# MoZhou1995/DeepPDE_ActorCritic

Hardware: AMD Instinct MI355X
Metric: SDE trajectory-steps/sec (batch×horizon) at d=20; value-fn rel-L2 vs analytic (higher is better)
Workload: dtype f32

## Files before the change

### deeppde_actorcritic_amd/csrc/dpac_device.h

```cpp
#pragma once

#include <hip/hip_runtime.h>
#include <rocrand/rocrand_kernel.h>
#include <stdint.h>

#include <type_traits>

#include "dpac.h"
#include "dpac_mfma.h"

namespace dpac {

__host__ __device__ constexpr int pow2_at_least(int v) {
  int p = 1;
  while (p < v) p *= 2;
  return p;
}
#ifndef DPAC_LANE_CAP
#define DPAC_LANE_CAP 16
#endif
#ifndef DPAC_LANE_COMPS
#define DPAC_LANE_COMPS 2
#endif
__host__ __device__ constexpr int lanes_for_dim(int D) {
// ... 216 lines not shown
  return __builtin_bit_cast(float, (unsigned)sw[0]) + __builtin_bit_cast(float, (unsigned)sw[1]);
}
__device__ __forceinline__ double row_pair_sum(double v) {
  const unsigned long long u = __builtin_bit_cast(unsigned long long, v);
  const unsigned lo = (unsigned)u, hi = (unsigned)(u >> 32);
  const auto sl = __builtin_amdgcn_permlane16_swap(lo, lo, false, false);
  const auto sh = __builtin_amdgcn_permlane16_swap(hi, hi, false, false);
  const double a = __builtin_bit_cast(double, ((unsigned long long)(unsigned)sh[0] << 32) | (unsigned)sl[0]);
  const double b = __builtin_bit_cast(double, ((unsigned long long)(unsigned)sh[1] << 32) | (unsigned)sl[1]);
  return a + b;
}

template <int P, typename T>
__device__ __forceinline__ T group_shift_in(T keep, T v, bool group_start) {
  if constexpr (P == 1) {
    return v;
  } else {
    constexpr int kRowShr1 = 0x111;
    T sh;
    if constexpr (sizeof(T) == 4) {
      sh = __builtin_bit_cast(T, __builtin_amdgcn_update_dpp(__builtin_bit_cast(int, v),
                                                            __builtin_bit_cast(int, keep),
                                                            kRowShr1, 0xF, 0xF, false));
    } else {
      const long long vb = __builtin_bit_cast(long long, v), kb = __builtin_bit_cast(long long, keep);
      const int lo = __builtin_amdgcn_update_dpp((int)vb, (int)kb, kRowShr1, 0xF, 0xF, false);
      const int hi = __builtin_amdgcn_update_dpp((int)(vb >> 32), (int)(kb >> 32), kRowShr1, 0xF, 0xF,
                                                 false);
      sh = __builtin_bit_cast(T, ((long long)hi << 32) | (unsigned int)lo);
    }
    if constexpr (P < 16) sh = group_start ? v : sh;
    return sh;
  }
}

template <typename T>
__device__ __forceinline__ void pin(T& v) {
  asm volatile("" : "+v"(v));
}
template <typename T, typename... Ts>
__device__ __forceinline__ void pin(T& v, Ts&... more) {
  pin(v);
  pin(more...);
}

template <int P>
struct Lanes {
  static_assert(P == 1 || P == 2 || P == 4 || P == 8 || P == 16 || P == 32, "bad group size");
  template <typename T>
  __device__ __forceinline__ static T sum(T v) {
    if constexpr (P >= 2) v = v + dpp<kDppXor1>(v);
    if constexpr (P >= 4) v = v + dpp<kDppXor2>(v);
    if constexpr (P >= 8) v = v + dpp<kDppHalfMirror>(v);
    if constexpr (P >= 16) v = v + dpp<kDppMirror>(v);
    if constexpr (P >= 32) v = row_pair_sum(v);
    return v;
  }
};

enum : uint64_t { kTagDw = 0, kTagDir = 1, kTagRadius = 2, kTagBdry = 3 };

__device__ __forceinline__ uint4 philox_block(uint64_t seed, uint64_t subseq, uint64_t block) {
  rocrand_state_philox4x32_10 st;
  rocrand_init(seed, subseq, block * 4ull, &st);
  return rocrand4(&st);
}

__device__ __forceinline__ void box_muller_hw(unsigned int x, unsigned int y, float& a, float& b) {
  const float u = ROCRAND_2POW32_INV + (x * ROCRAND_2POW32_INV);
  const float v = ROCRAND_2POW32_INV_2PI + (y * ROCRAND_2POW32_INV_2PI);
  const float s = __builtin_amdgcn_sqrtf(-2.0f * __logf(u));
  float sn, cs;
  __sincosf(v, &sn, &cs);
  a = sn * s;
  b = cs * s;
}
// ... 385 lines not shown
  __device__ __forceinline__ void drift_vjp(const T (&x)[M], const T (&u)[MC], T r, const T (&a)[M],
                            T (&gx)[M], T (&gu)[MC]) const {
#pragma unroll
    for (int i = 0; i < C; ++i) {
      const T x1 = x[i], x2 = x[C + i], a1 = a[i], a2v = a[C + i];
      gx[i] += a2v * (-2 * x1 * x2 - 1);
      gx[C + i] += a1 + a2v * (1 - x1 * x1);
      gu[i] += a2v;
    }
  }
  __device__ __forceinline__ void sigma_vjp(const T (&x)[M], const T (&u)[MC], const T (&a)[M], T (&gx)[M],
                            T (&gu)[MC]) const {}
  __device__ __forceinline__ void w_vjp(const T (&x)[M], const T (&u)[MC], T gw, T (&gx)[M], T (&gu)[MC]) const {
    T dv1[C], dv2[C], g[C], Ldv2[C], Lg[C];
    Lop(x, dv1);
    Lop(x + C, dv2);
#pragma unroll
    for (int i = 0; i < C; ++i) g[i] = (1 - x[i] * x[i]) * x[C + i] - x[i];
    Lop(dv2, Ldv2);
    Lop(g, Lg);
#pragma unroll
    for (int i = 0; i < C; ++i) {
      const T x1 = x[i], x2 = x[C + i];
      const T s1 = x[nxt(i)] + x[prv(i)], s2 = x[C + nxt(i)] + x[C + prv(i)];
      const T d1 = geps * s1 + 2 * x1 * x2 * dv2[i] + two_ga * x1;
      const T d2 = geps * s2 + Ldv2[i] * inv2q - dv1[i] - (1 - x1 * x1) * dv2[i] - Lg[i] + two_ga * x2;
      gx[i] += gw * d1;
      gx[C + i] += gw * d2;
      gu[i] += gw * (two_q * u[i]);
    }
  }
};

template <class E>
struct ConstSigma : std::false_type {};
template <typename T, int D, int P>
struct ConstSigma<EqLQR<T, D, P>> : std::true_type {};
template <typename T, int D, int P>
struct ConstSigma<EqEKN<T, D, P>> : std::true_type {};

}
```

### deeppde_actorcritic_amd/csrc/dpac_kernels.h

```cpp
#pragma once

#include <cmath>
#include <limits>
#include <type_traits>
#include <utility>

#include "dpac_device.h"

namespace dpac {

enum Op : int {
  OP_ROLLOUT = 0,
  OP_FLAG_INIT,
  OP_STEP_FWD,
  OP_STEP_BWD,
  OP_TD_FWD,
  OP_TD_BWD,
  OP_EVAL,
  OP_ROLLOUT_NN,
  OP_ROLLOUT_NN_BWD,
};

inline int nn_mask_tile_bytes(int n_hidden) { return 13 * 64 * n_hidden; }

struct OpArgs {
  int op;
  dpac_eqn_params eq;
  int scheme, dtype, td_type, cost_order, sample_type, what;
  int64_t B, traj_offset;
  int N;
  double T;
  uint64_t seed;
  const void *x0, *dw, *x, *u, *dt_in, *coef_in, *G, *disc_in, *y_in;
  const int32_t* flag_in;
  const void *g_x_out, *g_disc_out, *g_y_out;
  void *x_out, *dt, *coef, *u_out, *y, *disc, *disc_out, *y_out;
  int32_t* flag_out;
  void *g_x, *g_u, *g_disc, *g_G, *out;
  dpac_mlp mlp;
  void *save_z, *save_disc;
// ... 330 lines not shown
    if constexpr (WANT_U) su.store(rs_u, u, (uint32_t)t * slab_u);
    if constexpr (DPAC_ABLATE != 3) {
      constexpr int PH = decltype(phase)::value;
      keep = group_shift_in<P>(keep, tr.coef ? tr.dt : -tr.dt, lc.p == 0);
      if constexpr (PH >= 0) {
        if constexpr (PH % F == F - 1) flush(t, F);
      } else if ((t & (F - 1)) == F - 1) {
        flush(t, F);
      }
    }
  };
  pipelined<KB, DwFrame<T, M>>(0, a.N, load, body);
  if constexpr (DPAC_ABLATE != 3 && DPAC_ABLATE != 1 && DPAC_ABLATE != 5) {
    const int rem = a.N & (F - 1);
    if (rem) flush(a.N - 1, rem);
  }
  if constexpr (COST) {
    if (lc.live && lc.p == 0) {
      a.y[lc.b] = y;
      a.disc[lc.b] = disc;
    }
  }
}

#ifndef DPAC_ST_CHUNKS
#define DPAC_ST_CHUNKS 4
#endif
#ifndef DPAC_ST_TIGHT
#define DPAC_ST_TIGHT 0
#endif
#ifndef DPAC_ST_TIGHT_CHUNKS
#define DPAC_ST_TIGHT_CHUNKS 3
#endif
#ifndef DPAC_ST_PD
#define DPAC_ST_PD 1
#endif
constexpr int kStCW = 4;
constexpr int kStCH = 16;
constexpr int kStPD = DPAC_ST_PD;
#ifndef DPAC_ST_STEP
#define DPAC_ST_STEP 1
#endif
constexpr bool kOwnStep = DPAC_ST_STEP != 0;
static_assert(kStPD >= 1 && kStPD <= kStCH, "prefetch distance within a chunk");
template <typename T, int D, int P>
struct StagedPlan {
  static constexpr int TPW = kStCW * (64 / P);
  static constexpr int SLOT = TPW * D * (int)sizeof(T);
  static constexpr int PIECES = (SLOT + 1023) / 1024;
  static constexpr int kLdsCap = 128 * 1024;
  static constexpr int SLOT_1K = (SLOT + 16 + 1023) / 1024 * 1024;
  static constexpr int SLOT_16 = (SLOT + 16 + 15) / 16 * 16;
  static constexpr bool kWide = !DPAC_ST_TIGHT && DPAC_ST_CHUNKS * kStCH * SLOT_1K <= kLdsCap;
  static constexpr int CHUNKS = kWide ? DPAC_ST_CHUNKS : DPAC_ST_TIGHT_CHUNKS;
  static constexpr int SLOT_LDS = kWide ? SLOT_1K : SLOT_16;
  static constexpr int PADOFF = SLOT_LDS - 16;
  static constexpr int RS = CHUNKS * kStCH;
  static_assert(P < 4 || (SLOT % 16 == 0 && (PIECES - 1) * 1024 + 16 <= SLOT), "DMA pieces stay inside the slot");
  static constexpr bool kOk = P >= 4 && RS * SLOT_LDS <= kLdsCap && kStCH * PIECES <= 62;
};

template <class Fn, int... S>
__device__ __forceinline__ void unroll_phases(Fn& fn, std::integer_sequence<int, S...>) {
  (fn(Phase<S>{}), ...);
}

__device__ __forceinline__ int lds_load_relaxed(const int* p) {
  return __hip_atomic_load(p, __ATOMIC_RELAXED, __HIP_MEMORY_SCOPE_WORKGROUP);
}
__device__ __forceinline__ void lds_store_relaxed(int* p, int v) {
  __hip_atomic_store(p, v, __ATOMIC_RELAXED, __HIP_MEMORY_SCOPE_WORKGROUP);
}

template <int GEN>
constexpr int st_waves() { return kStCW + (GEN > 0 ? GEN : 1); }
#ifndef DPAC_ST_GEN
#define DPAC_ST_GEN 12
#endif
constexpr int kStGen = DPAC_ST_GEN;

#ifndef DPAC_ST_TRACE
#define DPAC_ST_TRACE 0
#endif
#if DPAC_ST_TRACE
constexpr int kStTraceRow = 128, kStTraceWaves = 16, kStTraceChunks = 32;
static __device__ uint32_t g_st_trace[2 * kStTraceWaves * kStTraceRow];
__device__ __forceinline__ uint32_t st_clock() {
  unsigned long long t;
  __builtin_amdgcn_sched_barrier(0);
  asm volatile("s_memtime %0\n\ts_waitcnt lgkmcnt(0)" : "=s"(t)::"memory");
  __builtin_amdgcn_sched_barrier(0);
  return (uint32_t)t;
}
__device__ __forceinline__ uint32_t st_realtime() {
  unsigned long long t;
  __builtin_amdgcn_sched_barrier(0);
  asm volatile("s_memrealtime %0\n\ts_waitcnt lgkmcnt(0)" : "=s"(t)::"memory");
  __builtin_amdgcn_sched_barrier(0);
  return (uint32_t)t;
}
#define ST_PUT(pt, v)                \
  do {                               \
    const uint32_t st_v_ = (v);      \
    if (st_on) st_row[(pt)] = st_v_; \
  } while (0)
#define ST_MARK(pt) ST_PUT(pt, st_clock())
#define ST_CHUNK(base, c0) ((base) + ((c0) / kStCH < kStTraceChunks ? (c0) / kStCH : kStTraceChunks - 1))
#else
#define ST_PUT(pt, v) \
  do {                \
  } while (0)
#define ST_MARK(pt) \
  do {              \
  } while (0)
#endif

template <typename T, class E, int D, int SCHEME, int OUT, int KB, int GEN = 0>
__global__ __launch_bounds__(64 * st_waves<GEN>()) void k_rollout_staged(const E eq, const DevConsts<T> c,
                                                                          const RolloutArgs<T> a) {
  constexpr int P = E::kP, M = E::M, MC = E::MC;
  using PL = StagedPlan<T, D, P>;
  constexpr int TPW = PL::TPW, RS = PL::RS, PIECES = PL::PIECES, SLOT_LDS = PL::SLOT_LDS;
  constexpr bool COST = (OUT & kOutCost) != 0, WANT_U = (OUT & kOutU) != 0;
  constexpr int F = P < kStCH ? P : kStCH;
  constexpr int NREADY = GEN > 0 ? GEN : 1;
  static_assert(kStCH % F == 0 && (F & (F - 1)) == 0, "flush phase fixed per unrolled body");
  static_assert(GEN == 0 || (2 * M <= 4 && kStCH % 2 == 0), "generators draw the paired layout");
  using TR = Transition<T, E, SCHEME>;
  __shared__ __attribute__((aligned(16))) unsigned char s_ring[RS * SLOT_LDS];
  __shared__ int s_ready[NREADY], s_done[kStCW];
  const int wave = __builtin_amdgcn_readfirstlane((int)threadIdx.x / 64), lane = (int)threadIdx.x % 64;
  const int64_t row0 = xcd_block(blockIdx.x, gridDim.x) * TPW;
  const int N = a.N;
#if DPAC_ST_TRACE
  const bool st_on = lane == 0 && wave < kStTraceWaves && (blockIdx.x == 0 || blockIdx.x == gridDim.x - 1);
  uint32_t* const st_row = g_st_trace + ((blockIdx.x == 0 ? 0 : kStTraceWaves) + (wave < kStTraceWaves ? wave : 0)) * kStTraceRow;
  ST_MARK(0);
  ST_PUT(5, st_realtime());
#endif
  if (threadIdx.x == 0) {
#pragma unroll
    for (int w = 0; w < NREADY; ++w) s_ready[w] = 0;
#pragma unroll
    for (int w = 0; w < kStCW; ++w) s_done[w] = 0;
  }
  if (threadIdx.x < RS * 4)
    reinterpret_cast<uint32_t*>(s_ring + (threadIdx.x / 4) * SLOT_LDS + PL::PADOFF)[threadIdx.x % 4] = 0u;
  __syncthreads();
  ST_MARK(1);

  if constexpr (GEN > 0) {
    if (wave >= kStCW) {
      const int g = wave - kStCW;
      const int64_t rows_live = (a.B - row0) < TPW ? (a.B - row0) : TPW;
      constexpr int PLS = (D + M - 1) / M;
      constexpr int NBLK = (kStCH / 2) * TPW * PLS;
      constexpr int PASSES = (NBLK + 64 * GEN - 1) / (64 * GEN);
      constexpr int SLOT_T = SLOT_LDS / (int)sizeof(T);
      T* const ringw = reinterpret_cast<T*>(s_ring);
      for (int c0 = 0; c0 < N; c0 += kStCH) {
        const int need = c0 + kStCH - RS;
        if (need > 0) {
          for (;;) {
            int mn = lds_load_relaxed(&s_done[0]);
#pragma unroll
            for (int w = 1; w < kStCW; ++w) mn = min(mn, lds_load_relaxed(&s_done[w]));
            if (mn >= need) break;
            __builtin_amdgcn_s_sleep(2);
          }
        }
        asm volatile("" ::: "memory");
#pragma unroll 1
        for (int k = 0; k < PASSES; ++k) {
          const int e = (k * GEN + g) * 64 + lane;
          const int u = e / (TPW * PLS), rem = e - u * (TPW * PLS);
          const int i = rem / PLS, p = rem - i * PLS;
          const int t0 = c0 + 2 * u;
          if (e < NBLK && t0 < N && i < rows_live) {
            T v[4];
            dw_block_values<T>(a.seed, (uint64_t)(a.traj_offset + row0 + i), (uint64_t)(t0 >> 1) * P + p,
                               a.sample_type, v);
            T* d0 = ringw + (t0 % RS) * SLOT_T + i * D + p * M;
            T* d1 = ringw + ((t0 + 1) % RS) * SLOT_T + i * D + p * M;
#pragma unroll
            for (int m = 0; m < M; ++m) {
              if (p * M + m < D) {
                d0[m] = v[m];
                if (t0 + 1 < N) d1[m] = v[M + m];
              }
            }
          }
        }
        asm volatile("s_waitcnt lgkmcnt(0)" ::: "memory");
        if (lane == 0) lds_store_relaxed(&s_ready[g], c0 + kStCH < N ? c0 + kStCH : N);
      }
      return;
    }
  } else if (wave == kStCW) {
    const int64_t rows_live = (a.B - row0) < TPW ? (a.B - row0) : TPW;
    const uint32_t bytes = (uint32_t)(rows_live * D * (int64_t)sizeof(T));
    const uint32_t lds0 = (uint32_t)(uintptr_t)(__attribute__((address_space(3))) unsigned char*)s_ring;
    const char* base = (const char*)(a.dw + row0 * D);
    const int64_t step_bytes = a.B * D * (int64_t)sizeof(T);
    for (int c0 = 0; c0 < N; c0 += kStCH) {
      const int need = c0 + kStCH - RS;
      if (need > 0) {
        for (;;) {
          int mn = lds_load_relaxed(&s_done[0]);
#pragma unroll
          for (int w = 1; w < kStCW; ++w) mn = min(mn, lds_load_relaxed(&s_done[w]));
          if (mn >= need) break;
          __builtin_amdgcn_s_sleep(2);
        }
      }
      asm volatile("" ::: "memory");
#if DPAC_ST_TRACE
      ST_MARK(ST_CHUNK(16, c0));
#endif
#pragma unroll
      for (int s = 0; s < kStCH; ++s) {
        const int t = c0 + s < N ? c0 + s : N - 1;
        const char* src = base + t * step_bytes;
        const uint32_t slot = lds0 + (uint32_t)((t % RS) * SLOT_LDS);
#pragma unroll
        for (int k = 0; k < PIECES; ++k) {
          const uint32_t off = (uint32_t)((k * 64 + lane) * 16);
          const char* gp = src + (off < bytes ? off : 0u);
          const uint32_t m0 = __builtin_amdgcn_readfirstlane(slot + (uint32_t)(k * 1024));
          if (off < bytes || lane == 0) {
            int keep;
            asm volatile("s_mov_b32 %0, m0\n\ts_mov_b32 m0, %2\n\ts_nop 0\n\tglobal_load_lds_dwordx4 %1, off\n\ts_mov_b32 m0, %0"
                         : "=&s"(keep) : "v"(gp), "s"(m0) : "memory");
          }
        }
      }
#if DPAC_ST_TRACE
      ST_MARK(ST_CHUNK(48, c0));
#endif
      if (c0 > 0) {
        asm volatile("s_waitcnt vmcnt(%0)" ::"n"(kStCH * PIECES) : "memory");
        if (lane == 0) lds_store_relaxed(&s_ready[0], c0);
#if DPAC_ST_TRACE
        ST_MARK(ST_CHUNK(80, c0));
#endif
      }
    }
    asm volatile("s_waitcnt vmcnt(0)" ::: "memory");
    if (lane == 0) lds_store_relaxed(&s_ready[0], N);
    ST_MARK(4);
    ST_PUT(6, st_realtime());
    return;
  }

  const LaneCoord<P> lc(a.B, lane, row0 + wave * (64 / P));
  const int gl = wave * (64 / P) + lane / P;
  const Own<D, P> own(lc.p);
  const Own<E::CDIM, P> ownu(lc.p);
  const BufSlab<T, D, P> sx(own, lc.b, lc.live);
  const BufSlab<T, E::CDIM, P> su(ownu, lc.b, lc.live);
  const uint32_t slab = (uint32_t)(a.B * D * sizeof(T));
  const uint32_t slab_u = (uint32_t)(a.B * E::CDIM * sizeof(T));
  const uint32_t row_bytes = (uint32_t)(N * sizeof(T));
  const __amdgpu_buffer_rsrc_t rs_x = make_rsrc(a.x, slab * (uint32_t)(N + 1));
  const __amdgpu_buffer_rsrc_t rs_u = make_rsrc(a.u, WANT_U ? slab_u * (uint32_t)N : 0u);
  const __amdgpu_buffer_rsrc_t rs_dt = make_rsrc(a.dt, (uint32_t)a.B * row_bytes);
  const __amdgpu_buffer_rsrc_t rs_cf = make_rsrc(a.coef, (uint32_t)a.B * row_bytes);
  const T* ring = reinterpret_cast<const T*>(s_ring);
  const int lds_e = gl * D + lc.p * M;
  constexpr bool kVecRead = Own<D, P>::kFull && (M * sizeof(T) == 8 || M * sizeof(T) == 16);
  const uint32_t lane_off = own.active() ? (uint32_t)(lds_e * (int)sizeof(T)) : (uint32_t)PL::PADOFF;
  T keep = 0;
  auto flush = [&](int t_last, int count) {
    const uint32_t off = (lc.live && lc.p < count)
                             ? (uint32_t)((lc.b * N + t_last - lc.p) * (int64_t)sizeof(T)) : kOOB;
    buf_store_scalar<T>(rs_dt, off, fabs(keep));
    buf_store_scalar<T>(rs_cf, off, keep > T(0) ? T(1) : T(0));
  };
  T x[M];
  sx.load(make_rsrc(a.x0, slab), x);
  sx.store(rs_x, x);
  T r = TR::kRadius ? dsqrt(Lanes<P>::sum(sumsq(x))) : T(0);
  Flags fl = SCHEME == DPAC_SCHEME_ADAPTIVE ? region(r, c) : Flags{true, false};
  T disc = 1, y = 0;
  T xc[M], rc = r;
#pragma unroll
  for (int m = 0; m < M; ++m) xc[m] = x[m];
  T Ra = fl.alive ? c.R : -std::numeric_limits<T>::infinity();
  bool alive = fl.alive;
  const T sq0 = SCHEME == DPAC_SCHEME_ADAPTIVE ? dsqrt(c.dt0) : c.sqrt_dt0;
  T dt = c.dt0, sq = sq0;
  if constexpr (kOwnStep && SCHEME == DPAC_SCHEME_ADAPTIVE) {
    dt = adaptive_dt_raw(fl.layer, r, c);
    dt = fl.layer ? fmax(dt, c.dt_min) : dt;
    sq = dsqrt(dt);
  }
  ST_MARK(2);
  auto read_dw_at = [&](int t, uint32_t slot_bytes, T (&dwv)[M]) {
    if constexpr (kVecRead) {
      typedef T vec __attribute__((ext_vector_type(M)));
      const vec v = *reinterpret_cast<const vec*>(s_ring + slot_bytes + lane_off);
#pragma unroll
      for (int m = 0; m < M; ++m) dwv[m] = v[m];
    } else {
      const T* slot = ring + (t % RS) * (SLOT_LDS / (int)sizeof(T)) + lds_e;
#pragma unroll
      for (int m = 0; m < M; ++m) dwv[m] = own.valid(m) ? slot[m] : T(0);
    }
  };
  auto read_dw = [&](int t, T (&dwv)[M]) { read_dw_at(t, (uint32_t)((t % RS) * SLOT_LDS), dwv); };
  auto body = [&](int t, const T (&dwv)[M], auto phase) {
    T u[MC];
    eq.u_true(x, r, u);
// ... 45 lines not shown
    } else {
      if constexpr (E::kNeedsNorm) rt = dsqrt(St);
      coef = alive && !(St - c.R2 >= T(0));
      alive = coef;
    }
    if constexpr (COST) {
      const T cf = coef ? T(1) : T(0);
      const T w = eq.w_finish(Lanes<P>::sum(eq.w_part(x, u)));
      y += cost_increment(a.cost_order, w, cf, dt, disc);
      disc = disc * disc_factor(dt, cf, c);
    }
    const T kv = coef ? dt : -dt;
#pragma unroll
    for (int m = 0; m < M; ++m) {
      x[m] = coef ? xt[m] : x[m];
      xc[m] = xt[m];
    }
    if constexpr (E::kNeedsNorm) {
      r = coef ? rt : r;
      rc = rt;
    }
    dt = dtn;
    sq = sqn;
    sx.template store<DPAC_ROLLOUT_X_AUX>(rs_x, x, (uint32_t)(t + 1) * slab);
    if constexpr (WANT_U) su.store(rs_u, u, (uint32_t)t * slab_u);
    constexpr int PH = decltype(phase)::value;
    keep = group_shift_in<P>(keep, kv, lc.p == 0);
    if constexpr (PH >= 0) {
      if constexpr (PH % F == F - 1) flush(t, F);
    } else if ((t & (F - 1)) == F - 1) {
      flush(t, F);
    }
  };
  for (int c0 = 0; c0 < N; c0 += kStCH) {
    const int want = c0 + kStCH < N ? c0 + kStCH : N;
#if DPAC_ST_TRACE
    const uint32_t st_poll0 = st_clock();
#endif
    for (;;) {
      int mn = lds_load_relaxed(&s_ready[0]);
#pragma unroll
      for (int w = 1; w < NREADY; ++w) mn = min(mn, lds_load_relaxed(&s_ready[w]));
      if (mn >= want) break;
      __builtin_amdgcn_s_sleep(1);
    }
    asm volatile("" ::: "memory");
#if DPAC_ST_TRACE
    {
      const uint32_t st_now = st_clock();
      ST_PUT(ST_CHUNK(16, c0), st_now);
      ST_PUT(ST_CHUNK(80, c0), st_now - st_poll0);
      if (c0 == 0) ST_PUT(3, st_now);
    }
#endif
    if (c0 + kStCH <= N) {
      const uint32_t cb = (uint32_t)__builtin_amdgcn_readfirstlane((c0 % RS) * SLOT_LDS);
      constexpr int PD = kStPD;
      T nxt[PD][M];
#pragma unroll
      for (int q = 0; q < PD; ++q) read_dw_at(c0 + q, cb + (uint32_t)(q * SLOT_LDS), nxt[q]);
      auto one = [&](auto sidx) {
        constexpr int S = decltype(sidx)::value;
        T cur[M];
#pragma unroll
        for (int m = 0; m < M; ++m) cur[m] = nxt[S % PD][m];
        if constexpr (S + PD < kStCH) read_dw_at(c0 + S + PD, cb + (uint32_t)((S + PD) * SLOT_LDS), nxt[S % PD]);
        if constexpr (PD > 1) __builtin_amdgcn_sched_barrier(0);
        if constexpr (kOwnStep)
          step(c0 + S, cur, Phase<S>{});
        else
          body(c0 + S, cur, Phase<S>{});
      };
      unroll_phases(one, std::make_integer_sequence<int, kStCH>{});
    } else {
      for (int t = c0; t < N; ++t) {
        T cur[M];
        read_dw(t, cur);
        if constexpr (kOwnStep)
          step(t, cur, Phase<-1>{});
        else
          body(t, cur, Phase<-1>{});
      }
    }
    asm volatile("s_waitcnt lgkmcnt(0)" ::: "memory");
    if (lane == 0) lds_store_relaxed(&s_done[wave], want);
#if DPAC_ST_TRACE
    ST_MARK(ST_CHUNK(48, c0));
#endif
  }
  const int rem = N & (F - 1);
  if (rem) flush(N - 1, rem);
#if DPAC_ST_TRACE
  ST_MARK(4);
  asm volatile("s_waitcnt vmcnt(0)" ::: "memory");
  ST_MARK(7);
  ST_PUT(6, st_realtime());
#endif
  if constexpr (COST) {
    if (lc.live && lc.p == 0) {
      a.y[lc.b] = y;
      a.disc[lc.b] = disc;
    }
  }
}

template <typename T, class E, int D, int SCHEME>
__global__ __launch_bounds__(64) void k_flag_init(const E eq, const DevConsts<T> c, int64_t B,
                                                   const T* x0, int32_t* flag) {
  constexpr int P = E::kP, M = E::M;
  const LaneCoord<P> lc(B, threadIdx.x, xcd_block(blockIdx.x, gridDim.x) * (64 / P));
  const Own<D, P> own(lc.p);
  T xv[M];
  own.load_masked(x0 + lc.b * D, xv);
  const T r = dsqrt(Lanes<P>::sum(sumsq(xv)));
  if (lc.p == 0) flag[lc.b] = SCHEME == DPAC_SCHEME_ADAPTIVE ? region(r, c).encode() : 1;
}

template <typename T>
struct StepArgs {
  int64_t B;
  int cost_order;
// ... 725 lines not shown
```

Measured before the change: 27.50 billion.

## Restructure staged rollout loader and consumer into grouped DMA issue with seamless chunk handoff

The loader wave now issues dw DMA in sub-groups of four steps using precomputed voffsets and a fast full-tile path that skips per-lane bounds checks and m0 save/restore. It also publishes readiness at finer granularity during the first chunks. The compute waves replace the per-chunk blocking poll with a seam loop that prefetches the next step's dw across chunk boundaries and polls readiness early. The aim is to shorten pipeline startup and hide chunk-boundary stalls, at the cost of more complex synchronisation and a requirement of at least three ring chunks. Some unused helpers are also removed.

Result: no change. 27.49 billion (-0.0%).

```diff
diff --git a/deeppde_actorcritic_amd/csrc/dpac_device.h b/deeppde_actorcritic_amd/csrc/dpac_device.h
--- a/deeppde_actorcritic_amd/csrc/dpac_device.h
+++ b/deeppde_actorcritic_amd/csrc/dpac_device.h
@@ -272,16 +272,6 @@
     if constexpr (P < 16) sh = group_start ? v : sh;
     return sh;
   }
-}
-
-template <typename T>
-__device__ __forceinline__ void pin(T& v) {
-  asm volatile("" : "+v"(v));
-}
-template <typename T, typename... Ts>
-__device__ __forceinline__ void pin(T& v, Ts&... more) {
-  pin(v);
-  pin(more...);
 }
 
 template <int P>
@@ -733,11 +723,4 @@
   }
 };
 
-template <class E>
-struct ConstSigma : std::false_type {};
-template <typename T, int D, int P>
-struct ConstSigma<EqLQR<T, D, P>> : std::true_type {};
-template <typename T, int D, int P>
-struct ConstSigma<EqEKN<T, D, P>> : std::true_type {};
-
-}
+}
diff --git a/deeppde_actorcritic_amd/csrc/dpac_kernels.h b/deeppde_actorcritic_amd/csrc/dpac_kernels.h
--- a/deeppde_actorcritic_amd/csrc/dpac_kernels.h
+++ b/deeppde_actorcritic_amd/csrc/dpac_kernels.h
@@ -6,6 +6,7 @@
 #include <utility>
 
 #include "dpac_device.h"
+#include "dpac_staged_sched.h"
 
 namespace dpac {
 
@@ -413,6 +414,18 @@
 #endif
 constexpr bool kOwnStep = DPAC_ST_STEP != 0;
 static_assert(kStPD >= 1 && kStPD <= kStCH, "prefetch distance within a chunk");
+#ifndef DPAC_ST_ISSUE
+#define DPAC_ST_ISSUE 1
+#endif
+#ifndef DPAC_ST_SUB
+#define DPAC_ST_SUB 1
+#endif
+#ifndef DPAC_ST_SEAM
+#define DPAC_ST_SEAM 1
+#endif
+constexpr bool kStIssue = DPAC_ST_ISSUE != 0, kStSub = DPAC_ST_SUB != 0, kStSeam = DPAC_ST_SEAM != 0;
+static_assert(stsched::kCH == kStCH, "the schedule header's chunk is the kernel's");
+static_assert(!kStSeam || kStPD == 1, "the seam loop carries one step of dw across the boundary");
 template <typename T, int D, int P>
 struct StagedPlan {
   static constexpr int TPW = kStCW * (64 / P);
@@ -448,6 +461,7 @@
 #define DPAC_ST_GEN 12
 #endif
 constexpr int kStGen = DPAC_ST_GEN;
+static_assert(64 * st_waves<kStGen>() <= 1024, "the Philox variant's workgroup (compute waves + generators) fits a 1024-thread block");
 
 #ifndef DPAC_ST_TRACE
 #define DPAC_ST_TRACE 0
@@ -496,6 +510,7 @@
   constexpr int NREADY = GEN > 0 ? GEN : 1;
   static_assert(kStCH % F == 0 && (F & (F - 1)) == 0, "flush phase fixed per unrolled body");
   static_assert(GEN == 0 || (2 * M <= 4 && kStCH % 2 == 0), "generators draw the paired layout");
+  static_assert(!kStSeam || stsched::ring_ok(PL::CHUNKS), "a wave waits for chunk c + 1 before it marks chunk c done");
   using TR = Transition<T, E, SCHEME>;
   __shared__ __attribute__((aligned(16))) unsigned char s_ring[RS * SLOT_LDS];
   __shared__ int s_ready[NREADY], s_done[kStCW];
@@ -567,54 +582,103 @@
       return;
     }
   } else if (wave == kStCW) {
+    using SC = stsched::Loader<PIECES, kStSub>;
+    constexpr int SUB = stsched::kSub, GROUPS = stsched::kGroups;
     const int64_t rows_live = (a.B - row0) < TPW ? (a.B - row0) : TPW;
     const uint32_t bytes = (uint32_t)(rows_live * D * (int64_t)sizeof(T));
     const uint32_t lds0 = (uint32_t)(uintptr_t)(__attribute__((address_space(3))) unsigned char*)s_ring;
-    const char* base = (const char*)(a.dw + row0 * D);
+    const char* const base = (const char*)(a.dw + row0 * D);
     const int64_t step_bytes = a.B * D * (int64_t)sizeof(T);
-    for (int c0 = 0; c0 < N; c0 += kStCH) {
-      const int need = c0 + kStCH - RS;
-      if (need > 0) {
-        for (;;) {
-          int mn = lds_load_relaxed(&s_done[0]);
-#pragma unroll
-          for (int w = 1; w < kStCW; ++w) mn = min(mn, lds_load_relaxed(&s_done[w]));
-          if (mn >= need) break;
-          __builtin_amdgcn_s_sleep(2);
-        }
-      }
-      asm volatile("" ::: "memory");
-#if DPAC_ST_TRACE
-      ST_MARK(ST_CHUNK(16, c0));
-#endif
-#pragma unroll
-      for (int s = 0; s < kStCH; ++s) {
-        const int t = c0 + s < N ? c0 + s : N - 1;
-        const char* src = base + t * step_bytes;
-        const uint32_t slot = lds0 + (uint32_t)((t % RS) * SLOT_LDS);
-#pragma unroll
-        for (int k = 0; k < PIECES; ++k) {
-          const uint32_t off = (uint32_t)((k * 64 + lane) * 16);
-          const char* gp = src + (off < bytes ? off : 0u);
-          const uint32_t m0 = __builtin_amdgcn_readfirstlane(slot + (uint32_t)(k * 1024));
-          if (off < bytes || lane == 0) {
-            int keep;
-            asm volatile("s_mov_b32 %0, m0\n\ts_mov_b32 m0, %2\n\ts_nop 0\n\tglobal_load_lds_dwordx4 %1, off\n\ts_mov_b32 m0, %0"
-                         : "=&s"(keep) : "v"(gp), "s"(m0) : "memory");
+    auto dma_fast = [](const char* src, uint32_t voff, uint32_t m0) {
+      asm volatile("s_mov_b32 m0, %2\n\ts_nop 0\n\tglobal_load_lds_dwordx4 %0, %1" ::"v"(voff), "s"(src), "s"(m0) : "memory");
+    };
+    auto dma_any = [&](const char* src, int k, uint32_t m0) {
+      const uint32_t off = (uint32_t)((k * 64 + lane) * 16);
+      const char* gp = src + (off < bytes ? off : 0u);
+      if (off < bytes || lane == 0) {
+        int keep;
+        asm volatile("s_mov_b32 %0, m0\n\ts_mov_b32 m0, %2\n\ts_nop 0\n\tglobal_load_lds_dwordx4 %1, off\n\ts_mov_b32 m0, %0"
+                     : "=&s"(keep) : "v"(gp), "s"(m0) : "memory");
+      }
+    };
+    auto run = [&](auto fast_tag) {
+      constexpr bool FAST = decltype(fast_tag)::value;
+      constexpr int LAST = PIECES - 1;
+      constexpr int LAST_LANES = (PL::SLOT - LAST * 1024) / 16;
+      uint32_t voff[PIECES];
+#pragma unroll
+      for (int k = 0; k < PIECES; ++k) voff[k] = (uint32_t)((k * 64 + lane) * 16);
+      const char* src = base;
+      int t = 0;
+      uint32_t slot = lds0;
+      for (int c = 0; c * kStCH < N; ++c) {
+        const int need = (c + 1) * kStCH - RS;
+        if (need > 0) {
+          for (;;) {
+            int mn = lds_load_relaxed(&s_done[0]);
+#pragma unroll
+            for (int w = 1; w < kStCW; ++w) mn = min(mn, lds_load_relaxed(&s_done[w]));
+            if (mn >= need) break;
+            __builtin_amdgcn_s_sleep(2);
           }
         }
-      }
+        asm volatile("" ::: "memory");
 #if DPAC_ST_TRACE
-      ST_MARK(ST_CHUNK(48, c0));
-#endif
-      if (c0 > 0) {
-        asm volatile("s_waitcnt vmcnt(%0)" ::"n"(kStCH * PIECES) : "memory");
-        if (lane == 0) lds_store_relaxed(&s_ready[0], c0);
+        ST_MARK(ST_CHUNK(16, c * kStCH));
+#endif
+#pragma unroll
+        for (int g = 0; g < GROUPS; ++g) {
+          asm volatile("s_waitcnt vmcnt(%0)" ::"n"(SC::kPre) : "memory");
+          const char* gsrc[SUB];
+          uint32_t gslot[SUB];
+#pragma unroll
+          for (int s = 0; s < SUB; ++s) {
+            gsrc[s] = src;
+            gslot[s] = slot;
+            ++t;
+            src += t < N ? step_bytes : 0;
+            slot += (uint32_t)SLOT_LDS;
+          }
+          if constexpr (FAST) {
+#pragma unroll
+            for (int k = 0; k < LAST + (LAST_LANES == 64 ? 1 : 0); ++k)
+#pragma unroll
+              for (int s = 0; s < SUB; ++s) dma_fast(gsrc[s], voff[k], gslot[s] + (uint32_t)(k * 1024));
+            if constexpr (LAST_LANES < 64) {
+              if (lane < LAST_LANES) {
+#pragma unroll
+                for (int s = 0; s < SUB; ++s) dma_fast(gsrc[s], voff[LAST], gslot[s] + (uint32_t)(LAST * 1024));
+              }
+            }
+          } else {
+#pragma unroll
+            for (int s = 0; s < SUB; ++s)
+#pragma unroll
+              for (int k = 0; k < PIECES; ++k) dma_any(gsrc[s], k, __builtin_amdgcn_readfirstlane(gslot[s] + (uint32_t)(k * 1024)));
+          }
 #if DPAC_ST_TRACE
-        ST_MARK(ST_CHUNK(80, c0));
-#endif
-      }
-    }
+          if (g == GROUPS - 1) ST_MARK(ST_CHUNK(48, c * kStCH));
+#endif
+          const int j = c * GROUPS + g;
+          if (SC::publishes(j)) {
+            asm volatile("s_waitcnt vmcnt(%0)" ::"n"(SC::kPost) : "memory");
+            const int p = SC::published(j);
+            if (lane == 0) lds_store_relaxed(&s_ready[0], p < N ? p : N);
+#if DPAC_ST_TRACE
+            if (g == GROUPS - 1)
+              ST_MARK(ST_CHUNK(80, c * kStCH));
+            else
+              ST_MARK(112 + g);
+#endif
+          }
+        }
+        if (slot == lds0 + (uint32_t)(RS * SLOT_LDS)) slot = lds0;
+      }
+    };
+    if (kStIssue && rows_live == TPW)
+      run(std::true_type{});
+    else
+      run(std::false_type{});
     asm volatile("s_waitcnt vmcnt(0)" ::: "memory");
     if (lane == 0) lds_store_relaxed(&s_ready[0], N);
     ST_MARK(4);
@@ -759,6 +823,7 @@
       flush(t, F);
     }
   };
+  if constexpr (!kStSeam)
   for (int c0 = 0; c0 < N; c0 += kStCH) {
     const int want = c0 + kStCH < N ? c0 + kStCH : N;
 #if DPAC_ST_TRACE
@@ -814,6 +879,96 @@
 #if DPAC_ST_TRACE
     ST_MARK(ST_CHUNK(48, c0));
 #endif
+  }
+  if constexpr (kStSeam) {
+    int seen = 0;
+#if DPAC_ST_TRACE
+    uint32_t st_blocked = 0;
+    ST_PUT(8, 1u);
+#endif
+    auto poll = [&]() {
+      int mn = lds_load_relaxed(&s_ready[0]);
+#pragma unroll
+      for (int w = 1; w < NREADY; ++w) mn = min(mn, lds_load_relaxed(&s_ready[w]));
+      return mn;
+    };
+    auto ensure = [&](int t) {
+      if (seen > t) return;
+#if DPAC_ST_TRACE
+      ++st_blocked;
+#endif
+      for (;;) {
+        seen = __builtin_amdgcn_readfirstlane(poll());
+        if (seen > t) break;
+        __builtin_amdgcn_s_sleep(1);
+      }
+      asm volatile("" ::: "memory");
+    };
+    const int nfull = N / kStCH;
+    uint32_t cb = 0;
+    T nxt[M];
+    if (nfull > 0) {
+      ensure(0);
+      ST_MARK(3);
+      read_dw_at(0, 0u, nxt);
+    }
+    auto chunk = [&](int c0, auto first_tag) {
+      constexpr bool FIRST = decltype(first_tag)::value;
+      const uint32_t cbe = cb + (uint32_t)(kStCH * SLOT_LDS);
+      const uint32_t cbn = cbe == (uint32_t)(RS * SLOT_LDS) ? 0u : cbe;
+      int early = 0;
+      auto one = [&](auto sidx) {
+        constexpr int S = decltype(sidx)::value;
+#if DPAC_ST_TRACE
+        if constexpr (S == 2) ST_MARK(ST_CHUNK(16, c0));
+        if constexpr (S == kStCH - 2) ST_MARK(ST_CHUNK(48, c0));
+#endif
+        T cur[M];
+#pragma unroll
+        for (int m = 0; m < M; ++m) cur[m] = nxt[m];
+        if constexpr (S == stsched::kPollAt) early = poll();
+        if constexpr (S + 1 < kStCH) {
+          if constexpr (FIRST && stsched::checks_ready(S + 1)) ensure(c0 + S + 1);
+          read_dw_at(c0 + S + 1, cb + (uint32_t)((S + 1) * SLOT_LDS), nxt);
+        } else {
+          const int e = __builtin_amdgcn_readfirstlane(early);
+          seen = e > seen ? e : seen;
+          asm volatile("" ::: "memory");
+          if (c0 + 2 * kStCH <= N) {
+            ensure(c0 + kStCH);
+            read_dw_at(c0 + kStCH, cbn, nxt);
+          }
+        }
+        if constexpr (kOwnStep)
+          step(c0 + S, cur, Phase<S>{});
+        else
+          body(c0 + S, cur, Phase<S>{});
+      };
+      unroll_phases(one, std::make_integer_sequence<int, kStCH>{});
+      asm volatile("" ::: "memory");
+      if (lane == 0) lds_store_relaxed(&s_done[wave], c0 + kStCH);
+#if DPAC_ST_TRACE
+      ST_PUT(ST_CHUNK(80, c0), st_blocked);
+      st_blocked = 0;
+#endif
+      cb = cbn;
+    };
+    if (nfull > 0) chunk(0, std::true_type{});
+    for (int c = 1; c < nfull; ++c) chunk(c * kStCH, std::false_type{});
+    if (nfull * kStCH < N) {
+      ensure(N - 1);
+      if (nfull == 0) ST_MARK(3);
+      for (int t = nfull * kStCH; t < N; ++t) {
+        T cur[M];
+        read_dw(t, cur);
+        if constexpr (kOwnStep)
+          step(t, cur, Phase<-1>{});
+        else
+          body(t, cur, Phase<-1>{});
+      }
+      asm volatile("" ::: "memory");
+      if (lane == 0) lds_store_relaxed(&s_done[wave], N);
+    }
   }
   const int rem = N & (F - 1);
   if (rem) flush(N - 1, rem);
diff --git a/deeppde_actorcritic_amd/csrc/dpac_staged_sched.h b/deeppde_actorcritic_amd/csrc/dpac_staged_sched.h
--- /dev/null
+++ b/deeppde_actorcritic_amd/csrc/dpac_staged_sched.h
@@ -0,0 +1,58 @@
+#pragma once
+
+namespace dpac {
+namespace stsched {
+
+constexpr int kCH = 16;
+constexpr int kSub = 4;
+constexpr int kGroups = kCH / kSub;
+constexpr int kVmMax = 62;
+static_assert(kCH % kSub == 0 && kGroups >= 2, "groups tile the chunk");
+
+template <int PIECES, bool SUB>
+struct Loader {
+  static constexpr int kGroupPieces = kSub * PIECES;
+  static constexpr int kPre = kVmMax - kGroupPieces;
+  static constexpr int kPost = kCH * PIECES;
+  static_assert(kPre >= 0 && kPost <= kVmMax, "a chunk's pieces fit in vmcnt");
+  static constexpr bool publishes(int j) {
+    if (j < kGroups) return false;
+    if (j % kGroups == kGroups - 1) return true;
+    return SUB && j < 2 * kGroups;
+  }
+  static constexpr int published(int j) { return (j + 1 - kGroups) * kSub; }
+  static constexpr int issued_pieces(int j) { return (j + 1) * kGroupPieces; }
+};
+
+constexpr int kPollAt = 8;
+static_assert(kPollAt >= 0 && kPollAt < kCH - 1, "the early poll is issued before the last step");
+constexpr bool checks_ready(int step_in_chunk) { return step_in_chunk % kSub == 0; }
+
+template <int PIECES, bool SUB>
+constexpr bool schedule_ok(int chunks) {
+  using L = Loader<PIECES, SUB>;
+  int out = 0, pub = 0;
+  for (int j = 0; j < chunks * kGroups; ++j) {
+    if (out > L::kPre) out = L::kPre;
+    out += L::kGroupPieces;
+    if (out > kVmMax) return false;
+    if (L::publishes(j)) {
+      if (out > L::kPost) out = L::kPost;
+      const int p = L::published(j);
+      if (p <= pub) return false;
+      if (p % kSub != 0) return false;
+      if (p * PIECES > L::issued_pieces(j) - L::kPost) return false;
+      pub = p;
+    }
+  }
+  return pub == (chunks - 1) * kCH;
+}
+static_assert(schedule_ok<1, true>(1) && schedule_ok<1, true>(2) && schedule_ok<1, true>(9), "PIECES = 1");
+static_assert(schedule_ok<2, true>(1) && schedule_ok<2, true>(2) && schedule_ok<2, true>(9), "PIECES = 2");
+static_assert(schedule_ok<3, true>(1) && schedule_ok<3, true>(2) && schedule_ok<3, true>(9), "PIECES = 3");
+static_assert(schedule_ok<2, false>(9) && schedule_ok<3, false>(9), "whole-chunk first hand-off");
+
+constexpr bool ring_ok(int chunks_in_ring) { return chunks_in_ring >= 3; }
+
+}
+}
```

## Cooperative first-chunk DMA and half-chunk double-buffered dW reads in staged rollout

Applied to the files above, without the earlier changes.

When the staged rollout runs without generator waves, the compute waves now DMA the first chunk of Brownian increments into LDS themselves, and the loader wave starts at the second chunk, joining the barrier late. The compute loop reads dW in two 8-step half batches, so one half is prefetched from LDS while the other is being stepped, and the ready check for the next chunk happens partway through. A constexpr model of the ring hand-off is added to check at compile time that reads stay behind ready and overwrites stay behind done, with no wait cycle. This costs more registers for the batch buffers and adds schedule complexity. Unused helpers are removed.

After: 27.59 billion before, 27.22 billion after. 1.4% lower.

```diff
diff --git a/deeppde_actorcritic_amd/csrc/dpac_device.h b/deeppde_actorcritic_amd/csrc/dpac_device.h
--- a/deeppde_actorcritic_amd/csrc/dpac_device.h
+++ b/deeppde_actorcritic_amd/csrc/dpac_device.h
@@ -272,16 +272,6 @@
     if constexpr (P < 16) sh = group_start ? v : sh;
     return sh;
   }
-}
-
-template <typename T>
-__device__ __forceinline__ void pin(T& v) {
-  asm volatile("" : "+v"(v));
-}
-template <typename T, typename... Ts>
-__device__ __forceinline__ void pin(T& v, Ts&... more) {
-  pin(v);
-  pin(more...);
 }
 
 template <int P>
@@ -733,11 +723,4 @@
   }
 };
 
-template <class E>
-struct ConstSigma : std::false_type {};
-template <typename T, int D, int P>
-struct ConstSigma<EqLQR<T, D, P>> : std::true_type {};
-template <typename T, int D, int P>
-struct ConstSigma<EqEKN<T, D, P>> : std::true_type {};
-
-}
+}
diff --git a/deeppde_actorcritic_amd/csrc/dpac_kernels.h b/deeppde_actorcritic_amd/csrc/dpac_kernels.h
--- a/deeppde_actorcritic_amd/csrc/dpac_kernels.h
+++ b/deeppde_actorcritic_amd/csrc/dpac_kernels.h
@@ -402,17 +402,105 @@
 #ifndef DPAC_ST_TIGHT_CHUNKS
 #define DPAC_ST_TIGHT_CHUNKS 3
 #endif
-#ifndef DPAC_ST_PD
-#define DPAC_ST_PD 1
-#endif
 constexpr int kStCW = 4;
 constexpr int kStCH = 16;
-constexpr int kStPD = DPAC_ST_PD;
+constexpr int kStHB = 8;
 #ifndef DPAC_ST_STEP
 #define DPAC_ST_STEP 1
 #endif
 constexpr bool kOwnStep = DPAC_ST_STEP != 0;
-static_assert(kStPD >= 1 && kStPD <= kStCH, "prefetch distance within a chunk");
+#ifndef DPAC_ST_COOP
+#define DPAC_ST_COOP 1
+#endif
+#ifndef DPAC_ST_PRE
+#define DPAC_ST_PRE 8
+#endif
+#ifndef DPAC_ST_PIPE
+#define DPAC_ST_PIPE 2
+#endif
+constexpr bool kStCoop = DPAC_ST_COOP != 0;
+constexpr int kStLag = kStCH;
+constexpr int kStPre = DPAC_ST_PRE, kStPipe = DPAC_ST_PIPE;
+static_assert(kStPre >= 0 && kStPre < kStCH && kStLag >= 1 && kStLag <= kStCH && kStPipe >= 0 && kStPipe <= 2, "knob ranges");
+static_assert(kStCH == 2 * kStHB && kStCH % kStCW == 0, "a chunk is two batches and splits evenly over the compute waves");
+
+constexpr int st_ready0(bool coop, int N) { return coop ? (N < kStCH ? N : kStCH) : 0; }
+constexpr int st_loader_first(bool coop) { return coop ? kStCH : 0; }
+constexpr int st_need_done(int c0, int RS) { return c0 + kStCH - RS; }
+constexpr int st_want_ready(int c0, int N) { return c0 + kStCH < N ? c0 + kStCH : N; }
+
+constexpr bool st_schedule_ok(int RS, int N, bool coop, int lag, bool seam) {
+  int ready = st_ready0(coop, N), done = 0;
+  int lt = st_loader_first(coop), lpart = 0;
+  bool lfin = false;
+  const int nfull = N / kStCH;
+  int cc = 0, cpart = 0, seen = 0;
+  bool cfin = false;
+  for (int it = 0; it < 16 * (N / kStCH + 2); ++it) {
+    bool moved = false;
+    if (!lfin) {
+      if (lt >= N) {
+        ready = N, lfin = true, moved = true;
+      } else {
+        const int need = st_need_done(lt, RS);
+        if (lpart == 0 ? (need <= 0 || done >= need) : true) {
+          const int first = lpart == 0 ? lt : lt + lag;
+          const int last = (lpart == 0 ? lt + lag : lt + kStCH) < N ? (lpart == 0 ? lt + lag : lt + kStCH) : N;
+          if (last > first && last - RS > (need > 0 ? need : 0)) return false;
+          if (lpart == 0 && last == lt + lag && lt > ready) ready = lt;
+          if (lpart == 1) lt += kStCH;
+          lpart ^= 1, moved = true;
+        }
+      }
+    }
+    if (!cfin) {
+      const int c0 = cc * kStCH;
+      if (cc < nfull) {
+        if (cpart == 0) {
+          if (cc > 0 && seam) {
+            cpart = 1, moved = true;
+          } else if (ready >= st_want_ready(c0, N)) {
+            seen = st_want_ready(c0, N);
+            if (seen < c0 + kStHB) return false;
+            cpart = 1, moved = true;
+          }
+        } else if (cpart == 1) {
+          if (seen < c0 + kStCH) return false;
+          done = c0 + kStCH, cpart = 2, moved = true;
+        } else if (seam && cc + 1 < nfull) {
+          if (ready >= st_want_ready(c0 + kStCH, N)) {
+            seen = st_want_ready(c0 + kStCH, N);
+            if (seen < c0 + kStCH + kStHB) return false;
+            ++cc, cpart = 0, moved = true;
+          }
+        } else {
+          ++cc, cpart = 0, moved = true;
+        }
+      } else if (c0 < N) {
+        if (ready >= N) done = N, cfin = true, moved = true;
+      } else {
+        cfin = true, moved = true;
+      }
+    }
+    if (lfin && cfin) return true;
+    if (!moved) return false;
+  }
+  return false;
+}
+constexpr bool st_schedule_ok_upto(int RS, int n0, int n1, bool coop, int lag, bool seam) {
+  for (int N = n0; N <= n1; ++N)
+    if (!st_schedule_ok(RS, N, coop, lag, seam)) return false;
+  return true;
+}
+#define DPAC_ST_PROVE(RS)                                                                              \
+  static_assert(st_schedule_ok_upto(RS, 1, RS, kStCoop, kStLag, kStPipe == 2) &&                       \
+                st_schedule_ok_upto(RS, RS + 1, 2 * RS, kStCoop, kStLag, kStPipe == 2) &&              \
+                st_schedule_ok_upto(RS, 2 * RS + 1, 3 * RS, kStCoop, kStLag, kStPipe == 2) &&          \
+                st_schedule_ok_upto(RS, 3 * RS + 1, 4 * RS, kStCoop, kStLag, kStPipe == 2),            \
+                "the staged hand-off: reads behind ready, overwrites behind done, no wait cycle")
+DPAC_ST_PROVE(DPAC_ST_CHUNKS * kStCH);
+DPAC_ST_PROVE(DPAC_ST_TIGHT_CHUNKS * kStCH);
+#undef DPAC_ST_PROVE
 template <typename T, int D, int P>
 struct StagedPlan {
   static constexpr int TPW = kStCW * (64 / P);
@@ -448,6 +536,7 @@
 #define DPAC_ST_GEN 12
 #endif
 constexpr int kStGen = DPAC_ST_GEN;
+static_assert(64 * st_waves<kStGen>() <= 1024, "a workgroup has at most 1024 threads");
 
 #ifndef DPAC_ST_TRACE
 #define DPAC_ST_TRACE 0
@@ -508,16 +597,29 @@
   ST_MARK(0);
   ST_PUT(5, st_realtime());
 #endif
+  constexpr bool kCoop = GEN == 0 && kStCoop;
+  static_assert(RS >= 2 * kStCH, "the loader's first chunk waits for no `done`");
   if (threadIdx.x == 0) {
 #pragma unroll
-    for (int w = 0; w < NREADY; ++w) s_ready[w] = 0;
+    for (int w = 0; w < NREADY; ++w) s_ready[w] = st_ready0(kCoop, N);
 #pragma unroll
     for (int w = 0; w < kStCW; ++w) s_done[w] = 0;
   }
   if (threadIdx.x < RS * 4)
     reinterpret_cast<uint32_t*>(s_ring + (threadIdx.x / 4) * SLOT_LDS + PL::PADOFF)[threadIdx.x % 4] = 0u;
-  __syncthreads();
-  ST_MARK(1);
+  if constexpr (!kCoop) {
+    __syncthreads();
+    ST_MARK(1);
+  }
+  const int64_t rows_live = (a.B - row0) < TPW ? (a.B - row0) : TPW;
+  const uint32_t dma_bytes = (uint32_t)(rows_live * D * (int64_t)sizeof(T));
+  const uint32_t lds0 = (uint32_t)(uintptr_t)(__attribute__((address_space(3))) unsigned char*)s_ring;
+  const int64_t step_bytes = a.B * D * (int64_t)sizeof(T);
+  auto dma16 = [&](const char* gp, uint32_t lds_dst) {
+    int keep;
+    asm volatile("s_mov_b32 %0, m0\n\ts_mov_b32 m0, %2\n\ts_nop 0\n\tglobal_load_lds_dwordx4 %1, off\n\ts_mov_b32 m0, %0"
+                 : "=&s"(keep) : "v"(gp), "s"(lds_dst) : "memory");
+  };
 
   if constexpr (GEN > 0) {
     if (wave >= kStCW) {
@@ -566,12 +668,80 @@
       }
       return;
     }
+  } else if constexpr (kCoop) {
+    if (wave == kStCW) {
+      constexpr int T0 = st_loader_first(kCoop);
+      const char* src = (const char*)(a.dw + row0 * D) + T0 * step_bytes;
+      bool joined = false;
+      auto join = [&]() {
+        asm volatile("s_waitcnt lgkmcnt(0)" ::: "memory");
+        __builtin_amdgcn_s_barrier();
+        asm volatile("" ::: "memory");
+        ST_MARK(1);
+      };
+      int published = st_ready0(kCoop, N);
+      for (int c0 = T0; c0 < N; c0 += kStCH) {
+        const int need = st_need_done(c0, RS);
+        if (need > 0) {
+          for (;;) {
+            int mn = lds_load_relaxed(&s_done[0]);
+#pragma unroll
+            for (int w = 1; w < kStCW; ++w) mn = min(mn, lds_load_relaxed(&s_done[w]));
+            if (mn >= need) break;
+            __builtin_amdgcn_s_sleep(2);
+          }
+        }
+        asm volatile("" ::: "memory");
+#if DPAC_ST_TRACE
+        ST_MARK(ST_CHUNK(16, c0));
+#endif
+        const uint32_t slot0 = lds0 + (uint32_t)((c0 % RS) * SLOT_LDS);
+        auto chunk = [&](auto whole) {
+#pragma unroll
+          for (int s = 0; s < kStCH; ++s) {
+            if (s == kStPre && !joined) {
+              join();
+              joined = true;
+            }
+            if (decltype(whole)::value || c0 + s < N) {
+#pragma unroll
+              for (int k = 0; k < PIECES; ++k) {
+                const uint32_t off = (uint32_t)((k * 64 + lane) * 16);
+                if (off < dma_bytes || lane == 0)
+                  dma16(src + (off < dma_bytes ? off : 0u), __builtin_amdgcn_readfirstlane(slot0 + (uint32_t)(s * SLOT_LDS + k * 1024)));
+              }
+              src += step_bytes;
+            }
+            if (s == kStLag - 1 && c0 > T0 && (decltype(whole)::value || c0 + s < N)) {
+              asm volatile("s_waitcnt vmcnt(%0)" ::"n"(kStLag * PIECES) : "memory");
+              if (lane == 0) lds_store_relaxed(&s_ready[0], c0);
+#if DPAC_ST_TRACE
+              if (published == st_ready0(kCoop, N)) ST_MARK(9);
+              ST_MARK(ST_CHUNK(80, c0));
+#endif
+              published = c0;
+            }
+          }
+        };
+        if (c0 + kStCH <= N)
+          chunk(std::true_type{});
+        else
+          chunk(std::false_type{});
+#if DPAC_ST_TRACE
+        ST_MARK(ST_CHUNK(48, c0));
+#endif
+      }
+      if (!joined) join();
+      asm volatile("s_waitcnt vmcnt(0)" ::: "memory");
+      if (lane == 0) lds_store_relaxed(&s_ready[0], N);
+      ST_MARK(4);
+      ST_PUT(6, st_realtime());
+      (void)published;
+      return;
+    }
   } else if (wave == kStCW) {
-    const int64_t rows_live = (a.B - row0) < TPW ? (a.B - row0) : TPW;
-    const uint32_t bytes = (uint32_t)(rows_live * D * (int64_t)sizeof(T));
-    const uint32_t lds0 = (uint32_t)(uintptr_t)(__attribute__((address_space(3))) unsigned char*)s_ring;
+    const uint32_t bytes = dma_bytes;
     const char* base = (const char*)(a.dw + row0 * D);
-    const int64_t step_bytes = a.B * D * (int64_t)sizeof(T);
     for (int c0 = 0; c0 < N; c0 += kStCH) {
       const int need = c0 + kStCH - RS;
       if (need > 0) {
@@ -648,6 +818,25 @@
   };
   T x[M];
   sx.load(make_rsrc(a.x0, slab), x);
+  if constexpr (kCoop) {
+    const char* base = (const char*)(a.dw + row0 * D);
+#pragma unroll
+    for (int s = 0; s < kStCH / kStCW; ++s) {
+      const int t = wave * (kStCH / kStCW) + s;
+      if (t < N) {
+#pragma unroll
+        for (int k = 0; k < PIECES; ++k) {
+          const uint32_t off = (uint32_t)((k * 64 + lane) * 16);
+          if (off < dma_bytes)
+            dma16(base + t * step_bytes + off, __builtin_amdgcn_readfirstlane(lds0 + (uint32_t)(t * SLOT_LDS + k * 1024)));
+        }
+      }
+    }
+    asm volatile("s_waitcnt vmcnt(0)" ::: "memory");
+    ST_MARK(8);
+    __syncthreads();
+    ST_MARK(1);
+  }
   sx.store(rs_x, x);
   T r = TR::kRadius ? dsqrt(Lanes<P>::sum(sumsq(x))) : T(0);
   Flags fl = SCHEME == DPAC_SCHEME_ADAPTIVE ? region(r, c) : Flags{true, false};
@@ -759,6 +948,103 @@
       flush(t, F);
     }
   };
+  auto ready_now = [&]() {
+    int mn = lds_load_relaxed(&s_ready[0]);
+#pragma unroll
+    for (int w = 1; w < NREADY; ++w) mn = min(mn, lds_load_relaxed(&s_ready[w]));
+    return mn;
+  };
+  auto run = [&](int t, const T (&cur)[M], auto phase) {
+    if constexpr (kOwnStep)
+      step(t, cur, phase);
+    else
+      body(t, cur, phase);
+  };
+  if constexpr (kStPipe > 0) {
+    const int nfull = N / kStCH;
+    T bA[kStHB][M], bB[kStHB][M];
+    auto read_batch = [&](int t0, uint32_t slot_bytes, T (&b)[kStHB][M]) {
+#pragma unroll
+      for (int q = 0; q < kStHB; ++q) read_dw_at(t0 + q, slot_bytes + (uint32_t)(q * SLOT_LDS), b[q]);
+    };
+    auto wait_ready = [&](int have, int want, int c0) {
+      if (have < want) {
+#if DPAC_ST_TRACE
+        const uint32_t st_poll0 = st_clock();
+#endif
+        while (ready_now() < want) __builtin_amdgcn_s_sleep(1);
+#if DPAC_ST_TRACE
+        ST_PUT(ST_CHUNK(80, c0), st_clock() - st_poll0);
+#endif
+      }
+      asm volatile("" ::: "memory");
+    };
+#if DPAC_ST_TRACE
+    for (int c = 0; c < kStTraceChunks; ++c) ST_PUT(80 + c, 0u);
+#endif
+    if (nfull > 0) {
+      wait_ready(st_ready0(kCoop, N), st_want_ready(0, N), 0);
+      ST_MARK(3);
+      read_batch(0, 0u, bA);
+    }
+    for (int c0 = 0; c0 + kStCH <= N; c0 += kStCH) {
+      const uint32_t cb = (uint32_t)__builtin_amdgcn_readfirstlane((c0 % RS) * SLOT_LDS);
+      const bool more = c0 + 2 * kStCH <= N;
+#if DPAC_ST_TRACE
+      ST_MARK(ST_CHUNK(16, c0));
+#endif
+      read_batch(c0 + kStHB, cb + (uint32_t)(kStHB * SLOT_LDS), bB);
+      int rdy = 0;
+      __builtin_amdgcn_sched_barrier(0);
+      auto first = [&](auto sidx) {
+        constexpr int S = decltype(sidx)::value;
+        if constexpr (kStPipe == 2 && S == kStHB / 2) rdy = ready_now();
+        run(c0 + S, bA[S], Phase<S>{});
+      };
+      unroll_phases(first, std::make_integer_sequence<int, kStHB>{});
+      asm volatile("s_waitcnt lgkmcnt(0)" ::: "memory");
+      if (lane == 0) lds_store_relaxed(&s_done[wave], c0 + kStCH);
+      if constexpr (kStPipe == 2) {
+        if (more) {
+          wait_ready(rdy, st_want_ready(c0 + kStCH, N), c0 + kStCH);
+          read_batch(c0 + kStCH, (uint32_t)__builtin_amdgcn_readfirstlane((int)((uint32_t)(c0 + kStCH) % RS) * SLOT_LDS), bA);
+        }
+      }
+      __builtin_amdgcn_sched_barrier(0);
+      auto second = [&](auto sidx) {
+        constexpr int S = decltype(sidx)::value;
+        run(c0 + kStHB + S, bB[S], Phase<kStHB + S>{});
+      };
+      unroll_phases(second, std::make_integer_sequence<int, kStHB>{});
+#if DPAC_ST_TRACE
+      ST_MARK(ST_CHUNK(48, c0));
+#endif
+      if constexpr (kStPipe == 1) {
+        if (more) {
+          wait_ready(0, st_want_ready(c0 + kStCH, N), c0 + kStCH);
+          read_batch(c0 + kStCH, (uint32_t)__builtin_amdgcn_readfirstlane((int)((uint32_t)(c0 + kStCH) % RS) * SLOT_LDS), bA);
+        }
+      }
+    }
+    if (nfull * kStCH < N) {
+      const int c0 = nfull * kStCH;
+#if DPAC_ST_TRACE
+      ST_MARK(ST_CHUNK(16, c0));
+#endif
+      wait_ready(0, N, c0);
+      if (nfull == 0) ST_MARK(3);
+      for (int t = c0; t < N; ++t) {
+        T cur[M];
+        read_dw(t, cur);
+        run(t, cur, Phase<-1>{});
+      }
+      asm volatile("s_waitcnt lgkmcnt(0)" ::: "memory");
+      if (lane == 0) lds_store_relaxed(&s_done[wave], N);
+#if DPAC_ST_TRACE
+      ST_MARK(ST_CHUNK(48, c0));
+#endif
+    }
+  } else
   for (int c0 = 0; c0 < N; c0 += kStCH) {
     const int want = c0 + kStCH < N ? c0 + kStCH : N;
 #if DPAC_ST_TRACE
@@ -782,7 +1068,7 @@
 #endif
     if (c0 + kStCH <= N) {
       const uint32_t cb = (uint32_t)__builtin_amdgcn_readfirstlane((c0 % RS) * SLOT_LDS);
-      constexpr int PD = kStPD;
+      constexpr int PD = 1;
       T nxt[PD][M];
 #pragma unroll
       for (int q = 0; q < PD; ++q) read_dw_at(c0 + q, cb + (uint32_t)(q * SLOT_LDS), nxt[q]);
@@ -792,7 +1078,6 @@
 #pragma unroll
         for (int m = 0; m < M; ++m) cur[m] = nxt[S % PD][m];
         if constexpr (S + PD < kStCH) read_dw_at(c0 + S + PD, cb + (uint32_t)((S + PD) * SLOT_LDS), nxt[S % PD]);
-        if constexpr (PD > 1) __builtin_amdgcn_sched_barrier(0);
         if constexpr (kOwnStep)
           step(c0 + S, cur, Phase<S>{});
         else
```
